# MachinaIO/mxx

Hardware: AMD Instinct MI355X
Metric: dcrt_ring_ops_per_s (higher is better)
Workload: dtype u32

## Files before the change

### mxx_amd/csrc/arith.hip

```cpp
#include "matmul_tile.h"

#include <algorithm>
#include <vector>

enum { OP_ADD = 0, OP_SUB = 1, OP_MUL = 2, OP_NEG = 3 };

template <typename W, int OP, bool BCAST, int VN>
__global__ void elementwise_kernel(W *__restrict__ out, const W *__restrict__ a, const W *__restrict__ b,
                                   const LimbConst *__restrict__ limbs, uint32_t L, uint32_t logN,
                                   size_t words_per_poly, size_t total_vecs) {
    size_t v = static_cast<size_t>(blockIdx.x) * blockDim.x + threadIdx.x;
    const size_t stride = static_cast<size_t>(gridDim.x) * blockDim.x;
    for (; v < total_vecs; v += stride) {
        const size_t w0 = v * VN;
        const uint32_t limb = static_cast<uint32_t>((w0 >> logN) % L);
        const LimbConst lc = limbs[limb];
        const W q = static_cast<W>(lc.q);
        const size_t bw0 = BCAST ? (w0 % words_per_poly) : w0;
        W av[VN], bv[VN], ov[VN];
        if (VN == 1) {
            av[0] = a[w0];
            bv[0] = b[bw0];
        } else {
            typedef typename std::conditional<sizeof(W) == 4, uint4, ulonglong2>::type V16;
// ... 439 lines not shown
            if (rc >= 0) return rc;
        }
        const bool want_dma = force ? (force == 'd' || force == 'w') : (rows32 && cols >= 16);
        if (want_dma) {
            const int rc = launch_matmul_dma_u32(out, lhs, rhs);
            if (rc >= 0) return rc;
        }
        const uint64_t lds_blocks = static_cast<uint64_t>(matrix_limbs(out)) * (N / 64) * ((cols + 15) / 16);
        const bool thin = rows <= 2 && cols >= 8 &&
                          lds_blocks <= 512 && (inner >= 128 || (rows >= 2 && inner >= 64));
        const bool want_lds = force ? (force == 'l' || force == 'd' || force == 'w') : ((rows >= 9 && cols >= 8 && !narrow) || thin);
        if (lds_ok && want_lds) return launch_matmul_lds_u32(out, lhs, rhs);
    }
    if (N >= 4) {
        switch (ctx->env.matmul_tile) {
#define MXX_TILE(R, C, S)                                                                   \
    case (R * 100 + C * 10 + S) * 2: return launch_matmul_cfg<uint32_t, R, C, S>(out, lhs, rhs); \
    case (R * 100 + C * 10 + S) * 2 + 1: return launch_matmul_cfg<uint32_t, R, C, S, true>(out, lhs, rhs);
            MXX_TILE(1, 8, 4) MXX_TILE(1, 4, 4) MXX_TILE(2, 8, 4) MXX_TILE(2, 4, 4) MXX_TILE(3, 4, 4) MXX_TILE(4, 4, 4)
            MXX_TILE(3, 8, 2) MXX_TILE(4, 8, 1) MXX_TILE(8, 8, 1) MXX_TILE(4, 8, 2)
#undef MXX_TILE
            default: break;
        }
        if (rows > 4 && rows <= 8) return launch_matmul_cfg<uint32_t, 8, 8, 1>(out, lhs, rhs);
        if (rows >= 4) {
            const uint64_t waves4 = static_cast<uint64_t>((N + 63) / 64) * ((cols + 7) / 8) * matrix_limbs(out);
            return waves4 <= 8192 ? launch_matmul_cfg<uint32_t, 4, 8, 1, true>(out, lhs, rhs) : launch_matmul_cfg<uint32_t, 4, 8, 1>(out, lhs, rhs);
        }
        if (rows == 3) {
            const uint64_t waves3 = static_cast<uint64_t>((N / 4 + 63) / 64) * ((cols + 3) / 4) * matrix_limbs(out);
            return waves3 <= 4096 ? launch_matmul_cfg<uint32_t, 3, 4, 4, true>(out, lhs, rhs) : launch_matmul_cfg<uint32_t, 3, 4, 4>(out, lhs, rhs);
        }
        const uint32_t tc = (rows >= 2 || cols >= 8) ? 8 : 4;
        const uint64_t tile_waves = static_cast<uint64_t>((N / 4 + 63) / 64) * ((rows + 1) / 2) * ((cols + tc - 1) / tc) * matrix_limbs(out);
        const bool ahead = tile_waves <= (rows >= 2 ? 1024u : 8192u);
        if (rows >= 2) return ahead ? launch_matmul_cfg<uint32_t, 2, 8, 4, true>(out, lhs, rhs) : launch_matmul_cfg<uint32_t, 2, 8, 4>(out, lhs, rhs);
        if (cols >= 8) {
            const int rc = launch_matmul_skinny24(out, lhs, rhs, ahead);
            if (rc >= 0) return rc;
        }
        if (cols >= 8) return ahead ? launch_matmul_cfg<uint32_t, 1, 8, 4, true>(out, lhs, rhs) : launch_matmul_cfg<uint32_t, 1, 8, 4>(out, lhs, rhs);
        return ahead ? launch_matmul_cfg<uint32_t, 1, 4, 4, true>(out, lhs, rhs) : launch_matmul_cfg<uint32_t, 1, 4, 4>(out, lhs, rhs);
    }
    return launch_matmul_cfg<uint32_t, 1, 4, 1>(out, lhs, rhs);
}

template <typename W, int OP, bool BCAST>
static int launch_elementwise_typed(GpuMatrix *out, const GpuMatrix *a, const GpuMatrix *b) {
    GpuContext *ctx = out->ctx;
    const size_t words = matrix_words(out);
    if (words == 0) return 0;
    const size_t wpp = matrix_limbs(out) * static_cast<size_t>(ctx->N);
    const uint32_t L = static_cast<uint32_t>(matrix_limbs(out));
    constexpr int VNATIVE = 16 / sizeof(W);
    MXX_TRACE_BYTES(static_cast<double>(words) * sizeof(W) * (1 + (OP == OP_NEG || BCAST || a == b ? 1 : 2)));
    if (ctx->N >= VNATIVE) {
        const size_t vecs = words / VNATIVE;
        unsigned blocks = static_cast<unsigned>(std::min<size_t>((vecs + 255) / 256, 16384));
        MXX_LAUNCH((elementwise_kernel<W, OP, BCAST, VNATIVE>), dim3(blocks), dim3(256), 0, ctx->stream,
                           static_cast<W *>(words_ptr(out)), static_cast<const W *>(words_ptr(a)),
                           static_cast<const W *>(words_ptr(b)), ctx->d_limbs, L, ctx->logN, wpp, vecs);
    } else {
        unsigned blocks = static_cast<unsigned>(std::min<size_t>((words + 255) / 256, 16384));
        MXX_LAUNCH((elementwise_kernel<W, OP, BCAST, 1>), dim3(blocks), dim3(256), 0, ctx->stream,
                           static_cast<W *>(words_ptr(out)), static_cast<const W *>(words_ptr(a)),
                           static_cast<const W *>(words_ptr(b)), ctx->d_limbs, L, ctx->logN, wpp, words);
    }
// ... 203 lines not shown
    if (out->ctx != lhs->ctx || out->ctx != rhs->ctx) return set_error(std::string(who) + ": context mismatch");
    if (out->level != lhs->level || out->level != rhs->level) return set_error(std::string(who) + ": level mismatch");
    if (mode != 0 && (base_bits == 0 || base_bits >= 63)) return set_error(std::string(who) + ": invalid base_bits");
    if (identity_size == 0) return set_error(std::string(who) + ": identity_size must be positive");
    if (storage_overlaps(out, lhs) || storage_overlaps(out, rhs)) return set_error(std::string(who) + ": output must not alias an input");
    GpuContext *ctx = out->ctx;
    const size_t L = matrix_limbs(out);
    const size_t dpt = mode == 0 ? 1 : (ctx->crt_bits + base_bits - 1) / base_bits;
    const size_t k = mode == 0 ? 1 : (mode == 1 ? dpt * L : dpt);
    const size_t w = rhs->rows * k;
    if (lhs->cols != w * identity_size || out->rows != lhs->rows || out->cols != rhs->cols * identity_size)
        return set_error(std::string(who) + ": shape mismatch");
    if (lhs->format != GPU_POLY_FORMAT_EVAL || (mode == 0 && rhs->format != GPU_POLY_FORMAT_EVAL))
        return set_error(std::string(who) + " requires Eval format");
    out->format = GPU_POLY_FORMAT_EVAL;
    if (matrix_polys(out) == 0) return 0;
    if (ctx_activate(ctx)) return 1;
    if (w == 0) {
        HIP_TRY(hipMemsetAsync(words_ptr(out), 0, out->bytes, ctx->stream));
        return 0;
    }
    const size_t poly_bytes = L * static_cast<size_t>(ctx->N) * ctx->word_bytes;
    size_t chunk = rhs->cols;
    if (mode != 0) {
        size_t free_b = 0, total_b = 0, budget = size_t(8) << 30;
        if (hipMemGetInfo(&free_b, &total_b) == hipSuccess) budget = std::max(budget, (free_b + ctx->cached_bytes) / 3);
        else (void)hipGetLastError();
        chunk = std::min(rhs->cols, std::max<size_t>(1, budget / (w * poly_bytes)));
    }
    const bool row_vector = lhs->rows == 1;
    const bool in_place = row_vector || (identity_size == 1 && chunk == rhs->cols);
    GpuMatrix *lhs_buf = nullptr, *prod = nullptr;
    int rc = 0;
    if (!row_vector && identity_size > 1) rc = gpu_matrix_create(ctx, out->level, lhs->rows, w, GPU_POLY_FORMAT_EVAL, &lhs_buf);
    if (!rc && !in_place) rc = gpu_matrix_create(ctx, out->level, lhs->rows, chunk, GPU_POLY_FORMAT_EVAL, &prod);
    for (size_t c0 = 0; !rc && c0 < rhs->cols; c0 += chunk) {
        const size_t cw = std::min(chunk, rhs->cols - c0);
        const bool whole = cw == rhs->cols;
        GpuMatrix *slice = nullptr, *dec = nullptr;
        if (!whole) {
            rc = gpu_matrix_create(ctx, out->level, rhs->rows, cw, rhs->format, &slice);
            if (!rc) rc = gpu_matrix_copy_block(slice, rhs, 0, 0, 0, c0, rhs->rows, cw);
        }
        const GpuMatrix *x = whole ? rhs : slice;
        if (!rc && mode != 0) {
            rc = gpu_matrix_create(ctx, out->level, w, cw, GPU_POLY_FORMAT_EVAL, &dec);
            if (!rc) rc = mode == 1 ? gpu_matrix_decompose_base(x, base_bits, dec) : gpu_matrix_decompose_base_small(x, base_bits, dec);
            x = dec;
        }
        for (size_t i = 0; !rc && i < identity_size; ++i) {
            GpuMatrix lhs_view = matrix_view(lhs, i * w, 1, w, poly_bytes);
            const GpuMatrix *a = lhs;
            if (row_vector) a = &lhs_view;
            else if (identity_size > 1) {
                rc = gpu_matrix_copy_block(lhs_buf, lhs, 0, 0, 0, i * w, lhs->rows, w);
                a = lhs_buf;
            }
            if (rc) break;
            if (row_vector) {
                GpuMatrix out_view = matrix_view(out, i * rhs->cols + c0, 1, cw, poly_bytes);
                rc = gpu_matrix_mul(&out_view, a, x);
            } else if (in_place) {
                rc = gpu_matrix_mul(out, a, x);
            } else {
                GpuMatrix prod_view = matrix_view(prod, 0, lhs->rows, cw, poly_bytes);
                rc = gpu_matrix_mul(&prod_view, a, x);
                if (!rc) rc = gpu_matrix_copy_block(out, &prod_view, 0, i * rhs->cols + c0, 0, 0, lhs->rows, cw);
            }
        }
        gpu_matrix_destroy(slice);
// ... 354 lines not shown
```

### mxx_amd/csrc/common.h

```cpp
#pragma once

#include <hip/hip_runtime.h>

#include <atomic>
#include <cstddef>
#include <cstdint>
#include <cstdio>
#include <exception>
#include <map>
#include <unordered_map>
#include <mutex>
#include <string>
#include <vector>

#include "../../include/gpupoly.h"

constexpr size_t GPUPOLY_MAX_LIMBS = 64;

struct LimbConst {
    uint64_t q;
    uint64_t mu;
    uint64_t mu64;
    uint64_t n_inv;
    uint64_t n_inv_sh;
// ... 2 lines not shown
    uint64_t inv_last_w_sh;
    uint32_t kbits;
    uint32_t lazy_terms;
};

struct EnvSwitches {
    int ntt_path = 0;
    int ntt14 = 0;
    bool decompose_fused = true;
    char matmul_path = 0;
    int matmul_tile = 0;
    bool gsamp_simple = false;
    bool gsamp_no_uni = false;
    bool p1_simple = false;
    int sampler_per_lane = 0;
    int sampler_fill_every = 0;
    bool ntt64_int = false;
    int ntt_phase = 0;
    bool serde_general = false;
    bool rng_compat = false;
    bool pack24 = true;
    int skinny24 = 0;
    int skinny24_shape = 0;
    size_t mul_decompose_many_budget = 0;
    size_t mul_decompose_pairs_budget = 0;
    size_t gadget_scalar_budget = 0;
    char mul_sum_path = 0;
    size_t crt_recompose_chunk_bytes = size_t(256) << 20;
    void load();
};

struct GpuContext {
    EnvSwitches env;
    int device = 0;
    std::vector<int> gpu_ids;
    uint32_t logN = 0;
    int N = 0;
    int level = 0;
    uint32_t dnum = 0;
    int limb_count = 0;
    bool wide = false;
    int word_bytes = 4;
    uint32_t crt_bits = 0;
    std::vector<uint64_t> moduli;
    hipStream_t stream = nullptr;
    LimbConst *d_limbs = nullptr;
// ... 30 lines not shown
};

struct LayoutTag {
    std::atomic<int> v{GPU_MATRIX_LAYOUT_WORDS};
    LayoutTag() = default;
    LayoutTag(const LayoutTag &o) : v(o.v.load(std::memory_order_acquire)) {}
    LayoutTag &operator=(const LayoutTag &o) {
        v.store(o.v.load(std::memory_order_acquire), std::memory_order_release);
        return *this;
    }
};

struct GpuMatrix {
    GpuContext *ctx = nullptr;
    int level = 0;
    size_t rows = 0, cols = 0;
    int format = GPU_POLY_FORMAT_EVAL;
    void *storage = nullptr;
    size_t bytes = 0;
    LayoutTag layout;
    bool borrowed = false;
    GpuMatrix *parent = nullptr;
    int views = 0;
};

struct GpuEventSet {
    std::vector<hipEvent_t> events;
    int device = 0;
    void *staging = nullptr;
    GpuContext *ctx = nullptr;
    void *dev_staging = nullptr;
};

struct GpuP1CovarianceCache {
    GpuContext *ctx = nullptr;
    int level = 0;
    size_t d = 0, m = 0, n = 0;
    double sigma = 0, s = 0, dgg_stddev = 0;
    double *sqrt_var = nullptr;
    double *update_coeff = nullptr;
    void *karney_div = nullptr;
};

struct P1KeyEntry {
    const double *sqrt_var;
    const double *update_coeff;
// ... 150 lines not shown
    void *release() {
        void *p = ptr;
        ptr = nullptr;
        return p;
    }
};
int matrix_check_same_shape(const GpuMatrix *a, const GpuMatrix *b, const char *who);
int coeff_domain_source(const GpuMatrix *mat, CtxBlock &scratch, const void **src);

int launch_ntt(GpuContext *ctx, void *data, size_t vectors, int limbs_per_poly, bool inverse);
int launch_ntt_lds_u32(GpuContext *ctx, uint32_t *data, size_t vectors, uint32_t L, bool inverse);
int launch_ntt_digits_u32(GpuContext *ctx, uint32_t *out, const uint32_t *coeff, size_t out_vectors, uint32_t L,
                          uint32_t src_cols, uint32_t towers, uint32_t dpt, uint32_t base_bits, size_t k, uint32_t td0 = 0);
int launch_ntt_lds_u64(GpuContext *ctx, uint64_t *data, size_t vectors, uint32_t L, bool inverse);
int launch_ntt_digits_u64(GpuContext *ctx, uint64_t *out, const uint64_t *coeff, size_t out_vectors, uint32_t L,
                          uint32_t src_cols, uint32_t towers, uint32_t dpt, uint32_t base_bits, size_t k, uint32_t td0 = 0);
int launch_intt_oop_u32(GpuContext *ctx, uint32_t *out, const uint32_t *in, size_t vectors, uint32_t L);
int launch_ntt_add_u32(GpuContext *ctx, uint32_t *out, const uint32_t *src, const uint32_t *add, size_t vectors, uint32_t L);
int launch_mul_intt_u32(GpuContext *ctx, uint32_t *out, const uint32_t *in, const uint32_t *w, size_t vectors, uint32_t L);
int launch_matmul(GpuMatrix *out, const GpuMatrix *lhs, const GpuMatrix *rhs);
int launch_ntt_fwd_pack24_u32(GpuContext *ctx, uint32_t *out, const uint32_t *in, size_t vectors, uint32_t L);
int launch_matmul_skinny24(GpuMatrix *out, const GpuMatrix *lhs, const GpuMatrix *rhs, bool small_grid);
int skinny24_parse_shape(const char *s);
int launch_matmul_dma_u32(GpuMatrix *out, const GpuMatrix *lhs, const GpuMatrix *rhs);
int launch_matmul_dma32_u32(GpuMatrix *out, const GpuMatrix *lhs, const GpuMatrix *rhs);
int launch_matmul_mfma_u32(GpuMatrix *out, const GpuMatrix *lhs, const GpuMatrix *rhs);
int launch_copy_block(GpuMatrix *out, const GpuMatrix *src, size_t dst_row, size_t dst_col, size_t src_row,
                      size_t src_col, size_t rows, size_t cols, bool add);
int sample_p1_keyed_segments(const GpuP1CovarianceCache *cache, const P1KeyEntry *d_keys, const GpuMatrix *tp2,
                             const GpuRngSeed *seeds, const size_t *seg_cols, size_t nseg, GpuMatrix *out);
int launch_scatter_i64(GpuMatrix *out, const int64_t *vals);
```

### mxx_amd/csrc/decompose.hip

```cpp
#include "common.h"
#include "modarith.h"

#include <algorithm>

static inline uint32_t host_bits(uint64_t v) { return v ? 64 - (uint32_t)__builtin_clzll(v) : 0; }

template <typename W>
__global__ void decompose_kernel(W *__restrict__ out, const W *__restrict__ src, const LimbConst *__restrict__ limbs,
                                 size_t src_polys, uint32_t src_cols, uint32_t L, uint32_t N, uint32_t towers,
                                 uint32_t dpt, uint32_t base_bits, size_t k) {
    const size_t idx = item_index();
    const size_t total = src_polys * towers * N;
    if (idx >= total) return;
    const uint32_t i = static_cast<uint32_t>(idx % N);
    const size_t pt = idx / N;
    const uint32_t t = static_cast<uint32_t>(pt % towers);
    const size_t p = pt / towers;
    const size_t r = p / src_cols, c = p - r * src_cols;
    const uint64_t residue = static_cast<uint64_t>(src[(p * L + t) * N + i]);
    const uint32_t src_bits = limbs[t].kbits;
    for (uint32_t d = 0; d < dpt; ++d) {
        const uint32_t shift = d * base_bits;
        uint64_t mask = 0;
        if (shift < src_bits) {
// ... 144 lines not shown

static int decompose_window(GpuContext *ctx, void *out, const void *coeff, size_t cols, size_t L, size_t k, uint32_t towers,
                            uint32_t dpt, uint32_t base_bits, size_t row_start, size_t R, bool eval) {
    const size_t row_bytes = cols * L * static_cast<size_t>(ctx->N) * static_cast<size_t>(ctx->word_bytes);
    char *o = static_cast<char *>(out);
    const char *c = static_cast<const char *>(coeff);
    const size_t first = row_start % k;
    size_t done = 0;
    if (first || R < k) {
        const size_t ky = std::min(R, k - first);
        if (int rc = decompose_segment(ctx, o, c, 1, cols, L, k, towers, dpt, base_bits, ky, static_cast<uint32_t>(first), eval)) return rc;
        done = ky;
        c += row_bytes;
    }
    if (const size_t whole = (R - done) / k) {
        if (int rc = decompose_segment(ctx, o + done * row_bytes, c, whole, cols, L, k, towers, dpt, base_bits, k, 0, eval)) return rc;
        done += whole * k;
        c += whole * row_bytes;
    }
    if (done < R) return decompose_segment(ctx, o + done * row_bytes, c, 1, cols, L, k, towers, dpt, base_bits, R - done, 0, eval);
    return 0;
}

static int decompose_core(const GpuMatrix *src, uint32_t base_bits, bool small, size_t row_start, GpuMatrix *out) {
    GpuContext *ctx = src->ctx;
    const int requested = out->format;
    const size_t L = matrix_limbs(src), R = out->rows, cols = src->cols;
    const uint32_t dpt = (ctx->crt_bits + base_bits - 1) / base_bits;
    const size_t k = small ? dpt : static_cast<size_t>(dpt) * L;
    if (R == 0 || cols == 0) {
        out->format = GPU_POLY_FORMAT_EVAL;
        return 0;
    }
    if (ctx_activate(ctx)) return 1;
    const size_t r0 = row_start / k, nsrc = (row_start + R - 1) / k - r0 + 1;
    const size_t row_bytes = cols * L * static_cast<size_t>(ctx->N) * static_cast<size_t>(ctx->word_bytes);
    const void *coeff = static_cast<const char *>(words_ptr(src)) + r0 * row_bytes;
    CtxBlock tmp_block(ctx);
    if (src->format == GPU_POLY_FORMAT_EVAL) {
        const size_t bytes = nsrc * row_bytes;
        if (tmp_block.alloc(bytes)) return 1;
        int rc = ctx->wide ? -1 : launch_intt_oop_u32(ctx, static_cast<uint32_t *>(tmp_block.ptr), static_cast<const uint32_t *>(coeff),
                                                      nsrc * cols * L, static_cast<uint32_t>(L));
        if (rc < 0) {
            MXX_TRACED_COPY("copy (device to device)", ctx->stream, 2.0 * bytes,
                            HIP_TRY(hipMemcpyAsync(tmp_block.ptr, coeff, bytes, hipMemcpyDeviceToDevice, ctx->stream)));
            rc = launch_ntt(ctx, tmp_block.ptr, nsrc * cols * L, static_cast<int>(L), true);
        }
        if (rc) return rc;
        coeff = tmp_block.ptr;
    }
    const uint32_t towers = small ? 1u : static_cast<uint32_t>(L);
    const bool eval = requested == GPU_POLY_FORMAT_EVAL;
    const int rc = decompose_window(ctx, words_ptr(out), coeff, cols, L, k, towers, dpt, base_bits, row_start - r0 * k, R, eval);
    if (rc == 0) out->format = eval ? GPU_POLY_FORMAT_EVAL : GPU_POLY_FORMAT_COEFF;
    return rc;
}

static int decompose_impl(const GpuMatrix *src, uint32_t base_bits, GpuMatrix *out, bool small) {
    if (!src || !out) return set_error("gpu_matrix_decompose_base: null matrix");
    if (base_bits == 0) return set_error("base_bits must be non-zero in gpu_matrix_decompose_base");
    if (src->ctx != out->ctx || src->level != out->level)
        return set_error("context mismatch in gpu_matrix_decompose_base");
    if (storage_overlaps(src, out)) return set_error("gpu_matrix_decompose_base: output must not alias the source");
    const size_t L = matrix_limbs(src);
    const uint32_t dpt = (src->ctx->crt_bits + base_bits - 1) / base_bits;
    const size_t k = small ? dpt : static_cast<size_t>(dpt) * L;
    if (out->rows != src->rows * k || out->cols != src->cols)
        return set_error("output size mismatch in gpu_matrix_decompose_base");
    return decompose_core(src, base_bits, small, 0, out);
}

extern "C" int gpu_matrix_fill_gadget(GpuMatrix *out, uint32_t base_bits) {
    ABI_GUARD_BEGIN
    return fill_gadget_impl(out, base_bits, false);
    ABI_GUARD_END
}

extern "C" int gpu_matrix_fill_small_gadget(GpuMatrix *out, uint32_t base_bits) {
    ABI_GUARD_BEGIN
    return fill_gadget_impl(out, base_bits, true);
    ABI_GUARD_END
}

extern "C" int gpu_matrix_decompose_base(const GpuMatrix *src, uint32_t base_bits, GpuMatrix *out) {
    ABI_GUARD_BEGIN
    return decompose_impl(src, base_bits, out, false);
    ABI_GUARD_END
}

extern "C" int gpu_matrix_decompose_base_small(const GpuMatrix *src, uint32_t base_bits, GpuMatrix *out) {
    ABI_GUARD_BEGIN
    return decompose_impl(src, base_bits, out, true);
// ... 198 lines not shown
```

### mxx_amd/csrc/layout.hip

```cpp
#include "common.h"

#include <stdexcept>

namespace {

__global__ void __launch_bounds__(256) unpack24_kernel(uint4 *__restrict__ words, const uint32_t *__restrict__ packed, size_t groups) {
    const size_t g = item_index();
    if (g >= groups) return;
    const uint32_t *p = packed + 3 * g;
    const uint32_t w0 = __builtin_nontemporal_load(p), w1 = __builtin_nontemporal_load(p + 1), w2 = __builtin_nontemporal_load(p + 2);
    words[g] = make_uint4(w0 & 0xffffffu, __builtin_amdgcn_alignbit(w1, w0, 24) & 0xffffffu,
                          __builtin_amdgcn_alignbit(w2, w1, 16) & 0xffffffu, w2 >> 8);
}

typedef uint32_t u32x4 __attribute__((ext_vector_type(4)));
__global__ void __launch_bounds__(256) pack24_kernel(uint32_t *__restrict__ packed, const u32x4 *__restrict__ words, size_t groups) {
    const size_t g = item_index();
    if (g >= groups) return;
    const u32x4 w = __builtin_nontemporal_load(words + g);
    uint32_t *p = packed + 3 * g;
    p[0] = w.x | (w.y << 24);
    p[1] = (w.y >> 8) | (w.z << 16);
    p[2] = (w.z >> 16) | (w.w << 8);
}
// ... 49 lines not shown
    GpuContext *ctx = m->ctx;
    const uint32_t L = static_cast<uint32_t>(matrix_limbs(m));
    const size_t vectors = matrix_polys(m) * L;
    std::unique_lock<std::mutex> lk(ctx->layout_mutex);
    if (m->views) {
        lk.unlock();
        return ntt ? launch_ntt(ctx, m->storage, vectors, static_cast<int>(L), false) : 0;
    }
    CtxBlock packed(ctx);
    if (packed.alloc(packed24_bytes(m))) return 1;
    int rc = ntt ? launch_ntt_fwd_pack24_u32(ctx, static_cast<uint32_t *>(packed.ptr), static_cast<const uint32_t *>(m->storage), vectors, L) : -1;
    if (rc < 0) {
        if (ntt && (rc = launch_ntt(ctx, m->storage, vectors, static_cast<int>(L), false))) return rc;
        const size_t groups = m->bytes / 16;
        MXX_TRACE_BYTES(static_cast<double>(packed24_bytes(m)) + m->bytes);
        MXX_LAUNCH(pack24_kernel, item_grid(groups, 256), dim3(256), 0, ctx->stream, static_cast<uint32_t *>(packed.ptr),
                   static_cast<const u32x4 *>(m->storage), groups);
        HIP_TRY(hipGetLastError());
    } else if (rc) {
        return rc;
    }
    ctx_free(ctx, m->storage);
    m->storage = packed.release();
    m->layout.v.store(GPU_MATRIX_LAYOUT_PACKED24, std::memory_order_release);
    return 0;
}
```

### mxx_amd/csrc/ntt14.h

```cpp
#pragma once

#include "ntt_lds.h"

namespace ntt14 {
constexpr int LOGN = 14;
constexpr uint32_t N = 1u << LOGN;
constexpr uint32_t T = 512;
constexpr int R0 = 32;
constexpr uint32_t BLK = 512;
constexpr uint32_t BLK_PAD = BLK + 64;
constexpr uint32_t GROUP_WORDS = 8 * BLK_PAD;

__device__ __forceinline__ uint32_t pad64(uint32_t pos) { return pos + ((pos >> 5) << 2); }

__device__ __forceinline__ void wave_sync() {
    __builtin_amdgcn_fence(__ATOMIC_ACQ_REL, "wavefront");
    __builtin_amdgcn_wave_barrier();
}

#ifdef GPUPOLY_PHASE_TIMING
#define NTT14_PHASE(bit) ((phase & (bit)) != 0)
#else
#define NTT14_PHASE(bit) false
#endif
// ... 187 lines not shown

template <typename W, bool TIGHT = false>
__global__ void __launch_bounds__(512, 8 / (sizeof(W) / 4))
    fwd_add_kernel(W *__restrict__ out, const W *__restrict__ src, const W *__restrict__ add,
                   const TwPair<W> *__restrict__ tw_all, const LimbConst *__restrict__ limbs, uint32_t L) {
    const uint32_t limb = blockIdx.x;
    const size_t vec = (static_cast<size_t>(blockIdx.z) * gridDim.y + blockIdx.y) * L + limb;
    const LimbConst lc = limbs[limb];
    fwd_body<W, TIGHT, true, LoadVector<W, true>, true, true>(out + vec * N, LoadVector<W, true>{src + vec * N}, tw_all, lc, limb, add + vec * N);
}

template <typename W, bool REDUCE>
struct LoadDigit {
    const W *src;
    uint32_t shift;
    W mask, q;
    __device__ __forceinline__ W operator()(uint32_t e) const {
        const W digit = (src[e] >> shift) & mask;
        if constexpr (REDUCE) return digit >= q ? digit % q : digit;
        else return digit;
    }
};

template <typename W, bool REDUCE, bool TIGHT = false, bool NTS = false>
__global__ void __launch_bounds__(512, 8 / (sizeof(W) / 4))
    fwd_digits_kernel(W *__restrict__ out, const W *__restrict__ coeff, const TwPair<W> *__restrict__ tw_all,
                      const LimbConst *__restrict__ limbs, uint32_t L, uint32_t src_cols, uint32_t towers, uint32_t dpt,
                      uint32_t base_bits, uint32_t k, uint32_t td0) {
    const uint32_t rest = blockIdx.x >> 3, col_hi = rest / L, limb = rest - col_hi * L;
    const uint32_t col = col_hi * 8u + (blockIdx.x & 7u);
    if (col >= src_cols) return;
    const uint32_t td = blockIdx.y + td0;
    const size_t r = blockIdx.z;
    const uint32_t t = td / dpt, d = td - t * dpt;
    const size_t vec = ((r * k + blockIdx.y) * src_cols + col) * L + limb;
    const LimbConst lc = limbs[limb];
    const uint32_t src_bits = limbs[t].kbits, shift = d * base_bits;
    LoadDigit<W, REDUCE> load;
    load.src = coeff + ((r * src_cols + col) * L + t) * N;
    load.shift = shift < 8 * sizeof(W) ? shift : 0;
    load.mask = 0;
    if (shift < src_bits && shift < 8 * sizeof(W)) {
        const uint32_t rem = src_bits - shift;
        const uint32_t db = base_bits < rem ? base_bits : rem;
        load.mask = db >= 8 * sizeof(W) ? static_cast<W>(~static_cast<W>(0)) : static_cast<W>((static_cast<W>(1) << db) - 1);
    }
    load.q = static_cast<W>(lc.q);
    (void)towers;
    fwd_body<W, TIGHT, NTS, LoadDigit<W, REDUCE>, false, NTS>(out + vec * N, load, tw_all, lc, limb);
}

template <typename W, bool SGN, bool MULW = false, int CAP = 31, int WPS = ((SGN && !MULW) ? 8 : 6), bool NT = false>
__global__ void __launch_bounds__(512, WPS / (sizeof(W) / 4))
    inv_kernel(W *__restrict__ data, const TwPair<W> *__restrict__ tw_all, const LimbConst *__restrict__ limbs,
               uint32_t L, const W *in = nullptr, const W *__restrict__ mulw = nullptr) {
    extern __shared__ __attribute__((aligned(16))) unsigned char smem[];
    W *xs = reinterpret_cast<W *>(smem);
    typedef typename std::conditional<sizeof(W) == 4, uint4, ulonglong2>::type V16;
    constexpr int VN = 16 / sizeof(W);
    const uint32_t tid = threadIdx.x, lane = tid & 63u;
    const uint32_t wave = __builtin_amdgcn_readfirstlane(tid >> 6);
    const uint32_t limb = blockIdx.x;
    const size_t vec = (static_cast<size_t>(blockIdx.z) * gridDim.y + blockIdx.y) * L + limb;
    const LimbConst lc = limbs[limb];
    const W q = static_cast<W>(lc.q);
    const W muw = static_cast<W>(sizeof(W) == 4 ? lc.mu32 : lc.mu64);
    const TwPair<W> *tw = tw_all + static_cast<size_t>(limb) * N;
    W *g = data + vec * N;
    const W *gin = (!MULW && in) ? in + vec * N : g;

    V16 dnext[8 / VN], wnext[8 / VN];
    const W *src0 = (MULW ? in + vec * N : g) + wave * BLK + 8 * lane;
// ... 95 lines not shown
```

### mxx_amd/csrc/ntt_lds_u32.hip

```cpp
#include "ntt_rings.h"

using W = uint32_t;

int launch_ntt_lds_u32(GpuContext *ctx, uint32_t *data, size_t vectors, uint32_t L, bool inverse) {
    return launch_ntt_lds<W>(ctx, data, vectors, L, inverse);
}

template __global__ void ntt14::inv_kernel<W, true, false, 31, 8, true>(W *, const TwPair<W> *, const LimbConst *, uint32_t, const W *,
                                                                        const W *);

template <typename R, bool TIGHT>
static int launch_lazy_mulw(GpuContext *ctx, W *out, const W *in, const W *w, size_t vectors, uint32_t L) {
    const size_t lds = R::template lds<W>();
    if (lds > kLdsLimitBytes) return -1;
    if (int rc = lds_opt_in<ntt_inv_lazy_kernel<W, R::LOGN, R::LOGR, R::WPE, 0, TIGHT, false, true>>(ctx, lds)) return rc;
    MXX_LAUNCH((ntt_inv_lazy_kernel<W, R::LOGN, R::LOGR, R::WPE, 0, TIGHT, false, true>), dim3(static_cast<unsigned>(vectors)), R::block(),
               lds, ctx->stream, out, tw_inv<W>(ctx), ctx->d_limbs_r, L, in, w);
    HIP_TRY(hipGetLastError());
    return 0;
}

template <typename R, bool TIGHT>
static int launch_split_mulw(GpuContext *ctx, W *out, const W *in, const W *w, size_t vectors, uint32_t L) {
    const size_t lds = R::template lds<W>();
// ... 59 lines not shown
    MXX_TRACE_BYTES(3.0 * vectors * ntt14::N * sizeof(W));
    return bool_dispatch(!ctx->lazy_ok, [&](auto TIGHT) {
        MXX_LAUNCH((ntt14::fwd_add_kernel<W, TIGHT()>), grid, dim3(ntt14::T), ntt14::lds_bytes(sizeof(W)), ctx->stream, out, src, add,
                   tw_fwd<W>(ctx), ctx->d_limbs, L);
        HIP_TRY(hipGetLastError());
        return 0;
    });
}

int launch_ntt_digits_u32(GpuContext *ctx, uint32_t *out, const uint32_t *coeff, size_t out_vectors, uint32_t L,
                          uint32_t src_cols, uint32_t towers, uint32_t dpt, uint32_t base_bits, size_t k, uint32_t td0) {
    DigitLaunch<W> d{out, coeff, L, src_cols, towers, dpt, base_bits, 0, td0};
    if (!ntt14_switches(ctx, true, true) || !d.plan(ctx, out_vectors, k)) return -1;
    MXX_TRACE_BYTES((static_cast<double>(d.src_rows) * src_cols * L + static_cast<double>(out_vectors)) * ctx->N * sizeof(W));
    if (ctx->logN != 14) return launch_ntt_digits<W>(ctx, d);
    const dim3 grid(8u * L * ((src_cols + 7u) / 8u), d.k, static_cast<unsigned>(d.src_rows));
    return bool_dispatch(d.reduce, !ctx->lazy_ok, d.nts, [&](auto RED, auto TIGHT, auto NTS) {
        MXX_LAUNCH((ntt14::fwd_digits_kernel<W, RED(), TIGHT(), NTS()>), grid, dim3(ntt14::T), ntt14::lds_bytes(sizeof(W)), ctx->stream, out,
                   coeff, tw_fwd<W>(ctx), ctx->d_limbs, L, src_cols, towers, dpt, base_bits, d.k, td0);
        HIP_TRY(hipGetLastError());
        return 0;
    });
}
```

### mxx_amd/csrc/runtime.hip

```cpp
#include "common.h"

#include <algorithm>
#include <cstdlib>
#include <iterator>
#include <map>
#include <cstring>
#include <dlfcn.h>

typedef unsigned __int128 u128h;

static thread_local std::string g_last_error;

int set_error(const char *msg) {
    g_last_error = msg ? msg : "unknown error";
    return 1;
}
int set_error(const std::string &msg) {
    g_last_error = msg;
    return 1;
}
int set_error(hipError_t err, const char *what) {
    g_last_error = std::string(what ? what : "hip call") + ": " + hipGetErrorString(err);
    (void)hipGetLastError();
    return 1;
// ... 223 lines not shown
    }
    if (const char *e = std::getenv("MXX_HIP_NTT14")) ntt14 = e[0] == 'w' ? 1 : (e[0] == 'u' ? 2 : 0);
    if (const char *e = std::getenv("MXX_HIP_DECOMPOSE_FUSED")) decompose_fused = e[0] != '0';
    if (const char *e = std::getenv("MXX_HIP_MATMUL_PATH")) matmul_path = e[0];
    if (const char *e = std::getenv("MXX_HIP_MATMUL_TILE")) {
        if (e[0] && e[1] && e[2]) matmul_tile = ((e[0] - '0') * 100 + (e[1] - '0') * 10 + (e[2] - '0')) * 2 + (e[3] == 'p');
    }
    if (const char *e = std::getenv("MXX_HIP_GSAMP")) {
        gsamp_simple = e[0] == 's';
        gsamp_no_uni = e[0] == 'n';
    }
    if (const char *e = std::getenv("MXX_HIP_P1")) p1_simple = e[0] == 's';
    if (const char *e = std::getenv("MXX_HIP_NTT64")) ntt64_int = e[0] == 'i';
    if (const char *e = std::getenv("MXX_HIP_RNG_COMPAT")) rng_compat = e[0] == 'r';
    if (const char *e = std::getenv("MXX_HIP_SERDE")) serde_general = e[0] == 'g';
    if (const char *e = std::getenv("MXX_HIP_PACK24")) pack24 = !(std::strcmp(e, "0") == 0 || std::strcmp(e, "off") == 0);
    if (const char *e = std::getenv("MXX_HIP_SKINNY24")) {
        if (std::strcmp(e, "0") == 0) skinny24 = 1;
        else if (std::strncmp(e, "force", 5) == 0 && (e[5] == 0 || e[5] == ':')) {
            skinny24 = 2;
            if (e[5] == ':') skinny24_shape = skinny24_parse_shape(e + 6) ? skinny24_parse_shape(e + 6) : -1;
        }
    }
    if (const char *e = std::getenv("MXX_HIP_MUL_DECOMPOSE_MANY_BUDGET")) mul_decompose_many_budget = static_cast<size_t>(std::strtoull(e, nullptr, 10));
    if (const char *e = std::getenv("MXX_HIP_MUL_DECOMPOSE_PAIRS_BUDGET")) mul_decompose_pairs_budget = static_cast<size_t>(std::strtoull(e, nullptr, 10));
    if (const char *e = std::getenv("MXX_HIP_GADGET_SCALAR_BUDGET")) gadget_scalar_budget = static_cast<size_t>(std::strtoull(e, nullptr, 10));
    if (const char *e = std::getenv("MXX_HIP_CRT_RECOMPOSE_CHUNK_BYTES")) {
        const size_t v = static_cast<size_t>(std::strtoull(e, nullptr, 10));
        if (v >= 1) crt_recompose_chunk_bytes = v;
    }
    if (const char *e = std::getenv("MXX_HIP_MUL_SUM_PATH")) mul_sum_path = (e[0] == 't' || e[0] == 's') ? e[0] : 0;
    if (const char *e = std::getenv("MXX_HIP_SAMPLER_PER_LANE")) {
        const int v = std::atoi(e);
        if (v >= 1 && v <= 4096) sampler_per_lane = v;
    }
    if (const char *e = std::getenv("MXX_HIP_NTT_PHASE")) {
        const int v = std::atoi(e);
        if (v >= 0 && v <= 127) ntt_phase = v;
    }
    if (const char *e = std::getenv("MXX_HIP_SAMPLER_FILL_EVERY")) {
        const int v = std::atoi(e);
        if (v >= 1 && v <= 8) sampler_fill_every = v;
    }
}

static std::mutex g_registry_mutex;
// ... 523 lines not shown
```

Baseline: 7.788 million.

## Emit decomposed digits in packed 24-bit layout and add few-row packed matmul kernel

In mul_decompose, the forward NTT of gadget digits now writes its output straight into a packed 3-byte-per-residue layout when the following matmul will read packed B, instead of producing full u32 digits that are later repacked. A new fewrow24 matmul kernel handles 4-8 row LHS against packed24 RHS, using either unaligned loads or ds_bpermute unpacking, with optional XCD-aware block remapping. The goal is to cut digit-matrix memory traffic and allocation by a quarter, allow larger chunks, and skip a separate pack pass. It adds considerable code and extra lane-shuffle work in the inner loop.

```diff
diff --git a/mxx_amd/csrc/arith.hip b/mxx_amd/csrc/arith.hip
--- a/mxx_amd/csrc/arith.hip
+++ b/mxx_amd/csrc/arith.hip
@@ -485,6 +485,10 @@
 #undef MXX_TILE
             default: break;
         }
+        if (rows >= 4 && rows <= 8) {
+            const int rc = launch_matmul_fewrow24(out, lhs, rhs);
+            if (rc >= 0) return rc;
+        }
         if (rows > 4 && rows <= 8) return launch_matmul_cfg<uint32_t, 8, 8, 1>(out, lhs, rhs);
         if (rows >= 4) {
             const uint64_t waves4 = static_cast<uint64_t>((N + 63) / 64) * ((cols + 7) / 8) * matrix_limbs(out);
@@ -506,6 +510,14 @@
         return ahead ? launch_matmul_cfg<uint32_t, 1, 4, 4, true>(out, lhs, rhs) : launch_matmul_cfg<uint32_t, 1, 4, 4>(out, lhs, rhs);
     }
     return launch_matmul_cfg<uint32_t, 1, 4, 1>(out, lhs, rhs);
+}
+
+bool matmul_reads_packed_b(const GpuContext *ctx, size_t rows, size_t inner, size_t cols, size_t L) {
+    const size_t N = static_cast<size_t>(ctx->N);
+    if (ctx->wide || ctx->env.matmul_path || ctx->env.matmul_tile || N < 64 || N % 64 || rows == 0 || rows > 8) return false;
+    const uint64_t lds_blocks = static_cast<uint64_t>(L) * (N / 64) * ((cols + 15) / 16);
+    const bool thin = rows <= 2 && cols >= 8 && lds_blocks <= 512 && (inner >= 128 || (rows >= 2 && inner >= 64));
+    return !thin;
 }
 
 template <typename W, int OP, bool BCAST>
@@ -755,11 +767,15 @@
     }
     const size_t poly_bytes = L * static_cast<size_t>(ctx->N) * ctx->word_bytes;
     size_t chunk = rhs->cols;
+    bool packed_d = false;
     if (mode != 0) {
         size_t free_b = 0, total_b = 0, budget = size_t(8) << 30;
         if (hipMemGetInfo(&free_b, &total_b) == hipSuccess) budget = std::max(budget, (free_b + ctx->cached_bytes) / 3);
         else (void)hipGetLastError();
-        chunk = std::min(rhs->cols, std::max<size_t>(1, budget / (w * poly_bytes)));
+        packed_d = !ctx->wide && ctx->pack24_ok && ctx->env.pack24 && (ctx->env.digits24 & 3) != 1 && ctx->logN == 14 &&
+                   matmul_reads_packed_b(ctx, lhs->rows, w, rhs->cols, L);
+        const size_t d_poly_bytes = packed_d ? poly_bytes / 4 * 3 : poly_bytes;
+        chunk = std::min(rhs->cols, std::max<size_t>(1, budget / (w * d_poly_bytes)));
     }
     const bool row_vector = lhs->rows == 1;
     const bool in_place = row_vector || (identity_size == 1 && chunk == rhs->cols);
@@ -777,8 +793,13 @@
         }
         const GpuMatrix *x = whole ? rhs : slice;
         if (!rc && mode != 0) {
-            rc = gpu_matrix_create(ctx, out->level, w, cw, GPU_POLY_FORMAT_EVAL, &dec);
-            if (!rc) rc = mode == 1 ? gpu_matrix_decompose_base(x, base_bits, dec) : gpu_matrix_decompose_base_small(x, base_bits, dec);
+            int prc = -1;
+            if (packed_d && matmul_reads_packed_b(ctx, lhs->rows, w, cw, L)) prc = decompose_base_packed24(x, base_bits, mode == 2, &dec);
+            if (prc >= 0) rc = prc;
+            else {
+                rc = gpu_matrix_create(ctx, out->level, w, cw, GPU_POLY_FORMAT_EVAL, &dec);
+                if (!rc) rc = mode == 1 ? gpu_matrix_decompose_base(x, base_bits, dec) : gpu_matrix_decompose_base_small(x, base_bits, dec);
+            }
             x = dec;
         }
         for (size_t i = 0; !rc && i < identity_size; ++i) {
diff --git a/mxx_amd/csrc/common.h b/mxx_amd/csrc/common.h
--- a/mxx_amd/csrc/common.h
+++ b/mxx_amd/csrc/common.h
@@ -48,6 +48,7 @@
     bool pack24 = true;
     int skinny24 = 0;
     int skinny24_shape = 0;
+    int digits24 = 0;
     size_t mul_decompose_many_budget = 0;
     size_t mul_decompose_pairs_budget = 0;
     size_t gadget_scalar_budget = 0;
@@ -124,6 +125,7 @@
     bool borrowed = false;
     GpuMatrix *parent = nullptr;
     int views = 0;
+    bool padded24 = false;
 };
 
 struct GpuEventSet {
@@ -320,6 +322,11 @@
 int launch_ntt_fwd_pack24_u32(GpuContext *ctx, uint32_t *out, const uint32_t *in, size_t vectors, uint32_t L);
 int launch_matmul_skinny24(GpuMatrix *out, const GpuMatrix *lhs, const GpuMatrix *rhs, bool small_grid);
 int skinny24_parse_shape(const char *s);
+int launch_matmul_fewrow24(GpuMatrix *out, const GpuMatrix *lhs, const GpuMatrix *rhs);
+bool matmul_reads_packed_b(const GpuContext *ctx, size_t rows, size_t inner, size_t cols, size_t L);
+int launch_ntt_digits_pack24_u32(GpuContext *ctx, uint32_t *out, const uint32_t *coeff, size_t out_vectors, uint32_t L,
+                                 uint32_t src_cols, uint32_t towers, uint32_t dpt, uint32_t base_bits, size_t k, bool probe);
+int decompose_base_packed24(const GpuMatrix *src, uint32_t base_bits, bool small, GpuMatrix **out);
 int launch_matmul_dma_u32(GpuMatrix *out, const GpuMatrix *lhs, const GpuMatrix *rhs);
 int launch_matmul_dma32_u32(GpuMatrix *out, const GpuMatrix *lhs, const GpuMatrix *rhs);
 int launch_matmul_mfma_u32(GpuMatrix *out, const GpuMatrix *lhs, const GpuMatrix *rhs);
diff --git a/mxx_amd/csrc/decompose.hip b/mxx_amd/csrc/decompose.hip
--- a/mxx_amd/csrc/decompose.hip
+++ b/mxx_amd/csrc/decompose.hip
@@ -190,6 +190,26 @@
     return 0;
 }
 
+static int coeff_rows(const GpuMatrix *src, size_t r0, size_t nsrc, CtxBlock &scratch, const void **coeff) {
+    GpuContext *ctx = src->ctx;
+    const size_t L = matrix_limbs(src), cols = src->cols;
+    const size_t row_bytes = cols * L * static_cast<size_t>(ctx->N) * static_cast<size_t>(ctx->word_bytes);
+    *coeff = static_cast<const char *>(words_ptr(src)) + r0 * row_bytes;
+    if (src->format != GPU_POLY_FORMAT_EVAL) return 0;
+    const size_t bytes = nsrc * row_bytes;
+    if (scratch.alloc(bytes)) return 1;
+    int rc = ctx->wide ? -1 : launch_intt_oop_u32(ctx, static_cast<uint32_t *>(scratch.ptr), static_cast<const uint32_t *>(*coeff),
+                                                  nsrc * cols * L, static_cast<uint32_t>(L));
+    if (rc < 0) {
+        MXX_TRACED_COPY("copy (device to device)", ctx->stream, 2.0 * bytes,
+                        HIP_TRY(hipMemcpyAsync(scratch.ptr, *coeff, bytes, hipMemcpyDeviceToDevice, ctx->stream)));
+        rc = launch_ntt(ctx, scratch.ptr, nsrc * cols * L, static_cast<int>(L), true);
+    }
+    if (rc) return rc;
+    *coeff = scratch.ptr;
+    return 0;
+}
+
 static int decompose_core(const GpuMatrix *src, uint32_t base_bits, bool small, size_t row_start, GpuMatrix *out) {
     GpuContext *ctx = src->ctx;
     const int requested = out->format;
@@ -202,22 +222,9 @@
     }
     if (ctx_activate(ctx)) return 1;
     const size_t r0 = row_start / k, nsrc = (row_start + R - 1) / k - r0 + 1;
-    const size_t row_bytes = cols * L * static_cast<size_t>(ctx->N) * static_cast<size_t>(ctx->word_bytes);
-    const void *coeff = static_cast<const char *>(words_ptr(src)) + r0 * row_bytes;
+    const void *coeff = nullptr;
     CtxBlock tmp_block(ctx);
-    if (src->format == GPU_POLY_FORMAT_EVAL) {
-        const size_t bytes = nsrc * row_bytes;
-        if (tmp_block.alloc(bytes)) return 1;
-        int rc = ctx->wide ? -1 : launch_intt_oop_u32(ctx, static_cast<uint32_t *>(tmp_block.ptr), static_cast<const uint32_t *>(coeff),
-                                                      nsrc * cols * L, static_cast<uint32_t>(L));
-        if (rc < 0) {
-            MXX_TRACED_COPY("copy (device to device)", ctx->stream, 2.0 * bytes,
-                            HIP_TRY(hipMemcpyAsync(tmp_block.ptr, coeff, bytes, hipMemcpyDeviceToDevice, ctx->stream)));
-            rc = launch_ntt(ctx, tmp_block.ptr, nsrc * cols * L, static_cast<int>(L), true);
-        }
-        if (rc) return rc;
-        coeff = tmp_block.ptr;
-    }
+    if (int rc = coeff_rows(src, r0, nsrc, tmp_block, &coeff)) return rc;
     const uint32_t towers = small ? 1u : static_cast<uint32_t>(L);
     const bool eval = requested == GPU_POLY_FORMAT_EVAL;
     const int rc = decompose_window(ctx, words_ptr(out), coeff, cols, L, k, towers, dpt, base_bits, row_start - r0 * k, R, eval);
@@ -237,6 +244,46 @@
     if (out->rows != src->rows * k || out->cols != src->cols)
         return set_error("output size mismatch in gpu_matrix_decompose_base");
     return decompose_core(src, base_bits, small, 0, out);
+}
+
+int decompose_base_packed24(const GpuMatrix *src, uint32_t base_bits, bool small, GpuMatrix **out) {
+    *out = nullptr;
+    GpuContext *ctx = src->ctx;
+    if (ctx->wide || !ctx->env.pack24 || (ctx->env.digits24 & 3) == 1) return -1;
+    const size_t L = matrix_limbs(src), cols = src->cols;
+    const uint32_t dpt = (ctx->crt_bits + base_bits - 1) / base_bits;
+    const size_t k = small ? dpt : static_cast<size_t>(dpt) * L;
+    const uint32_t towers = small ? 1u : static_cast<uint32_t>(L);
+    const size_t out_vectors = src->rows * k * cols * L;
+    if (out_vectors == 0 || cols >> 32 ||
+        launch_ntt_digits_pack24_u32(ctx, nullptr, nullptr, out_vectors, static_cast<uint32_t>(L), static_cast<uint32_t>(cols), towers, dpt,
+                                     base_bits, k, true) < 0)
+        return -1;
+    if (ctx_activate(ctx)) return 1;
+    const void *coeff = nullptr;
+    CtxBlock tmp_block(ctx);
+    if (int rc = coeff_rows(src, 0, src->rows, tmp_block, &coeff)) return rc;
+    GpuMatrix *m = new GpuMatrix();
+    m->ctx = ctx;
+    m->level = src->level;
+    m->rows = src->rows * k;
+    m->cols = cols;
+    m->format = GPU_POLY_FORMAT_EVAL;
+    m->bytes = matrix_words(m) * static_cast<size_t>(ctx->word_bytes);
+    if (ctx_alloc(ctx, packed24_bytes(m) + 16, &m->storage)) {
+        delete m;
+        return 1;
+    }
+    m->padded24 = true;
+    m->layout.v.store(GPU_MATRIX_LAYOUT_PACKED24, std::memory_order_release);
+    const int rc = launch_ntt_digits_pack24_u32(ctx, static_cast<uint32_t *>(m->storage), static_cast<const uint32_t *>(coeff), out_vectors,
+                                                static_cast<uint32_t>(L), static_cast<uint32_t>(cols), towers, dpt, base_bits, k, false);
+    if (rc) {
+        gpu_matrix_destroy(m);
+        return rc < 0 ? set_error("gpupoly_matrix_mul_decompose: the packed digit transform refused a launch it had accepted") : rc;
+    }
+    *out = m;
+    return 0;
 }
 
 extern "C" int gpu_matrix_fill_gadget(GpuMatrix *out, uint32_t base_bits) {
diff --git a/mxx_amd/csrc/layout.hip b/mxx_amd/csrc/layout.hip
--- a/mxx_amd/csrc/layout.hip
+++ b/mxx_amd/csrc/layout.hip
@@ -95,6 +95,7 @@
     }
     ctx_free(ctx, m->storage);
     m->storage = packed.release();
+    m->padded24 = false;
     m->layout.v.store(GPU_MATRIX_LAYOUT_PACKED24, std::memory_order_release);
     return 0;
 }
diff --git a/mxx_amd/csrc/matmul_fewrow24.hip b/mxx_amd/csrc/matmul_fewrow24.hip
--- /dev/null
+++ b/mxx_amd/csrc/matmul_fewrow24.hip
@@ -0,0 +1,160 @@
+#include "common.h"
+#include "matmul_tile.h"
+#include "modarith.h"
+
+#include <string>
+
+namespace fewrow24 {
+
+typedef uint32_t u32_unaligned __attribute__((aligned(1)));
+
+template <int TR, bool NTB, int LD>
+__global__ void __launch_bounds__(256)
+    kernel(uint32_t *__restrict__ C, const uint32_t *__restrict__ A, const unsigned char *__restrict__ B, const LimbConst *__restrict__ limbs,
+           uint32_t rows, uint32_t inner, uint32_t cols, uint32_t L, uint32_t N, uint32_t col_tiles, uint32_t share) {
+    constexpr int TC = 8;
+    uint32_t limb, bx, by;
+    if (share) {
+        const uint32_t xcd = blockIdx.x & 7u, j = blockIdx.x >> 3, xblocks = N / 256u;
+        by = j % col_tiles;
+        const uint32_t group = (j / col_tiles) * 8u + xcd;
+        limb = group / xblocks;
+        bx = group - limb * xblocks;
+    } else {
+        limb = blockIdx.z;
+        bx = blockIdx.x;
+        by = blockIdx.y;
+    }
+    const uint32_t rt = by / col_tiles, ct = by - rt * col_tiles;
+    const uint32_t r0 = rt * TR, c0 = ct * TC;
+    const uint32_t i = bx * blockDim.x + threadIdx.x;
+    const LimbConst lc = limbs[limb];
+    const uint32_t q = static_cast<uint32_t>(lc.q);
+    const uint32_t lane = threadIdx.x & 63u;
+
+    const size_t strideA = static_cast<size_t>(L) * N;
+    size_t a_off[TR], b_off[TC];
+#pragma unroll
+    for (int r = 0; r < TR; ++r) {
+        const uint32_t rr = min(r0 + r, rows - 1);
+        a_off[r] = (static_cast<size_t>(rr) * inner * L + limb) * N + i;
+    }
+    const uint32_t lane_off = LD == 0 ? i * 3u : (i - lane) * 3u + min(lane, 47u) * 4u;
+#pragma unroll
+    for (int c = 0; c < TC; ++c) {
+        const uint32_t cc = min(c0 + c, cols - 1);
+        b_off[c] = (static_cast<size_t>(cc) * L + limb) * N * 3 + lane_off;
+    }
+    const size_t strideBk = static_cast<size_t>(cols) * L * N * 3;
+    const uint32_t d = (lane * 3u) >> 2, sh = ((lane * 3u) & 3u) * 8u;
+    const int sel_lo = static_cast<int>(d * 4u), sel_hi = static_cast<int>(min(d + 1u, 47u) * 4u);
+
+    uint64_t acc[TR][TC];
+#pragma unroll
+    for (int r = 0; r < TR; ++r)
+#pragma unroll
+        for (int c = 0; c < TC; ++c) acc[r][c] = 0;
+    const uint32_t lazy = lc.lazy_terms;
+    uint32_t pending = 0;
+    for (uint32_t k = 0; k < inner; ++k) {
+        uint32_t av[TR], bv[TC];
+#pragma unroll
+        for (int r = 0; r < TR; ++r) av[r] = A[a_off[r] + k * strideA];
+#pragma unroll
+        for (int c = 0; c < TC; ++c) {
+            const unsigned char *p = B + b_off[c] + k * strideBk;
+            if constexpr (LD == 0) {
+                const u32_unaligned *src = reinterpret_cast<const u32_unaligned *>(p);
+                if constexpr (NTB) bv[c] = __builtin_nontemporal_load(src);
+                else bv[c] = *src;
+            } else {
+                const uint32_t *src = reinterpret_cast<const uint32_t *>(p);
+                if constexpr (NTB) bv[c] = __builtin_nontemporal_load(src);
+                else bv[c] = *src;
+            }
+        }
+#pragma unroll
+        for (int c = 0; c < TC; ++c) {
+            if constexpr (LD == 0) {
+                bv[c] &= 0xffffffu;
+            } else {
+                const uint32_t lo = static_cast<uint32_t>(__builtin_amdgcn_ds_bpermute(sel_lo, static_cast<int>(bv[c])));
+                const uint32_t hi = static_cast<uint32_t>(__builtin_amdgcn_ds_bpermute(sel_hi, static_cast<int>(bv[c])));
+                bv[c] = __builtin_amdgcn_alignbit(hi, lo, sh) & 0xffffffu;
+            }
+        }
+#pragma unroll
+        for (int r = 0; r < TR; ++r)
+#pragma unroll
+            for (int c = 0; c < TC; ++c) acc[r][c] += static_cast<uint64_t>(av[r]) * static_cast<uint64_t>(bv[c]);
+        if (++pending == lazy) {
+            pending = 0;
+#pragma unroll
+            for (int r = 0; r < TR; ++r)
+#pragma unroll
+                for (int c = 0; c < TC; ++c) acc[r][c] = reduce_u64_sum(acc[r][c], q, lc.mu64);
+        }
+    }
+#pragma unroll
+    for (int r = 0; r < TR; ++r) {
+        if (r0 + r >= rows) continue;
+#pragma unroll
+        for (int c = 0; c < TC; ++c) {
+            if (c0 + c >= cols) continue;
+            C[((static_cast<size_t>(r0 + r) * cols + (c0 + c)) * L + limb) * N + i] = reduce_u64_sum(acc[r][c], q, lc.mu64);
+        }
+    }
+}
+
+constexpr int kDefaultLoader = 1;
+
+}
+
+int launch_matmul_fewrow24(GpuMatrix *out, const GpuMatrix *lhs, const GpuMatrix *rhs) {
+    using namespace fewrow24;
+    GpuContext *ctx = out->ctx;
+    const EnvSwitches &env = ctx->env;
+    const int form = env.digits24 & 3;
+    if (form == 1 || ctx->wide || lhs->ctx != ctx || rhs->ctx != ctx) return -1;
+    const uint32_t rows = static_cast<uint32_t>(lhs->rows), inner = static_cast<uint32_t>(lhs->cols), cols = static_cast<uint32_t>(rhs->cols);
+    const uint32_t L = static_cast<uint32_t>(matrix_limbs(out)), N = static_cast<uint32_t>(ctx->N);
+    if (lhs->rows < 4 || lhs->rows > 8 || N % 256 != 0) return -1;
+    if (rhs->layout.v.load(std::memory_order_acquire) != GPU_MATRIX_LAYOUT_PACKED24) return -1;
+    const bool tall = rows > 4;
+    if (!tile_grid_fits(rows, cols, tall ? 8 : 4, 8)) return set_error("gpu_matrix_mul: matrix too large");
+    const TileGrid g = tall ? tile_grid<8, 8, 1>(ctx, rows, cols, L, rhs->bytes) : tile_grid<4, 8, 1>(ctx, rows, cols, L, rhs->bytes);
+    const int ld = rhs->padded24 ? (form == 2 ? 0 : (form == 3 ? 1 : kDefaultLoader)) : 1;
+    uint32_t *c = static_cast<uint32_t *>(words_ptr(out));
+    if (lhs->layout.v.load(std::memory_order_acquire) == GPU_MATRIX_LAYOUT_PACKED24) (void)words_ptr(lhs);
+    std::lock_guard<std::mutex> lk(ctx->layout_mutex);
+    bool pa = false, pb = false;
+    const uint32_t *a = static_cast<const uint32_t *>(packed24_ptr(lhs, &pa));
+    const unsigned char *b = static_cast<const unsigned char *>(packed24_ptr(rhs, &pb));
+    if (pa || !pb) return -1;
+    auto label = [](int key) {
+        const int tr = key & 4 ? 8 : 4, ld_ = key & 1;
+        const bool nt = key & 2;
+        return "fewrow24::kernel<TR=" + std::to_string(tr) + (nt ? ",nt" : "") + (ld_ ? ",bpermute" : ",unaligned") +
+               ",packed24 B> (the tile of matmul_kernel<u32," + std::to_string(tr) + ",8,1>, one slot per lane, 3-byte residues, " +
+               (ld_ ? "48 aligned dwords per wave through ds_bpermute" : "one unaligned dword per lane") +
+               (nt ? ", B streamed once with non-temporal loads)" : ")");
+    };
+    static const std::string name[8] = {label(0), label(1), label(2), label(3), label(4), label(5), label(6), label(7)};
+    const int key = (tall ? 4 : 0) | (g.streamed ? 2 : 0) | ld;
+    MXX_TRACE_BYTES(static_cast<double>(lhs->bytes) + packed24_bytes(rhs) + out->bytes);
+    const uint64_t blocks = static_cast<uint64_t>(g.grid.x) * g.grid.y * g.grid.z;
+    const uint32_t share = (env.digits24 & 4) == 0 && g.col_tiles > 1 && (static_cast<uint64_t>(L) * (N / 256u)) % 8 == 0 && blocks <= 0x7fffffffull;
+    const dim3 grid = share ? dim3(static_cast<unsigned>(blocks)) : g.grid;
+#define MXX_FR(KEY_)                                                                                                                        \
+    case KEY_:                                                                                                                          \
+        MXX_LAUNCH((kernel<(KEY_ & 4 ? 8 : 4), (KEY_ & 2) != 0, (KEY_ & 1)>), grid, dim3(g.threads), 0, ctx->stream, c, a, b, ctx->d_limbs, \
+                   rows, inner, cols, L, N, g.col_tiles, share);                                                                       \
+        break;
+    switch (key) {
+        MXX_FR(0) MXX_FR(1) MXX_FR(2) MXX_FR(3) MXX_FR(4) MXX_FR(5) MXX_FR(6) MXX_FR(7)
+    }
+#undef MXX_FR
+    ctx->last_kernel = name[key].c_str();
+    HIP_TRY(hipGetLastError());
+    return 0;
+}
diff --git a/mxx_amd/csrc/ntt14.h b/mxx_amd/csrc/ntt14.h
--- a/mxx_amd/csrc/ntt14.h
+++ b/mxx_amd/csrc/ntt14.h
@@ -233,7 +233,7 @@
     }
 };
 
-template <typename W, bool REDUCE, bool TIGHT = false, bool NTS = false>
+template <typename W, bool REDUCE, bool TIGHT = false, bool NTS = false, bool PK = false>
 __global__ void __launch_bounds__(512, 8 / (sizeof(W) / 4))
     fwd_digits_kernel(W *__restrict__ out, const W *__restrict__ coeff, const TwPair<W> *__restrict__ tw_all,
                       const LimbConst *__restrict__ limbs, uint32_t L, uint32_t src_cols, uint32_t towers, uint32_t dpt,
@@ -258,7 +258,7 @@
     }
     load.q = static_cast<W>(lc.q);
     (void)towers;
-    fwd_body<W, TIGHT, NTS, LoadDigit<W, REDUCE>, false, NTS>(out + vec * N, load, tw_all, lc, limb);
+    fwd_body<W, TIGHT, NTS, LoadDigit<W, REDUCE>, false, NTS, false, PK>(out + vec * (PK ? N / 4 * 3 : N), load, tw_all, lc, limb);
 }
 
 template <typename W, bool SGN, bool MULW = false, int CAP = 31, int WPS = ((SGN && !MULW) ? 8 : 6), bool NT = false>
diff --git a/mxx_amd/csrc/ntt_lds_u32.hip b/mxx_amd/csrc/ntt_lds_u32.hip
--- a/mxx_amd/csrc/ntt_lds_u32.hip
+++ b/mxx_amd/csrc/ntt_lds_u32.hip
@@ -105,3 +105,18 @@
         return 0;
     });
 }
+
+int launch_ntt_digits_pack24_u32(GpuContext *ctx, uint32_t *out, const uint32_t *coeff, size_t out_vectors, uint32_t L,
+                                 uint32_t src_cols, uint32_t towers, uint32_t dpt, uint32_t base_bits, size_t k, bool probe) {
+    DigitLaunch<W> d{nullptr, coeff, L, src_cols, towers, dpt, base_bits, 0, 0};
+    if (ctx->logN != 14 || !ctx->pack24_ok || !ctx->lazy_ok || !ntt14_switches(ctx, false, true) || !d.plan(ctx, out_vectors, k)) return -1;
+    if (probe) return 0;
+    MXX_TRACE_BYTES((static_cast<double>(d.src_rows) * src_cols * L + 0.75 * static_cast<double>(out_vectors)) * ctx->N * sizeof(W));
+    const dim3 grid(8u * L * ((src_cols + 7u) / 8u), d.k, static_cast<unsigned>(d.src_rows));
+    return bool_dispatch(d.reduce, d.nts, [&](auto RED, auto NTS) {
+        MXX_LAUNCH((ntt14::fwd_digits_kernel<W, RED(), false, NTS(), true>), grid, dim3(ntt14::T), ntt14::lds_bytes(sizeof(W)), ctx->stream, out,
+                   coeff, tw_fwd<W>(ctx), ctx->d_limbs, L, src_cols, towers, dpt, base_bits, d.k, 0u);
+        HIP_TRY(hipGetLastError());
+        return 0;
+    });
+}
diff --git a/mxx_amd/csrc/runtime.hip b/mxx_amd/csrc/runtime.hip
--- a/mxx_amd/csrc/runtime.hip
+++ b/mxx_amd/csrc/runtime.hip
@@ -269,6 +269,8 @@
             if (e[5] == ':') skinny24_shape = skinny24_parse_shape(e + 6) ? skinny24_parse_shape(e + 6) : -1;
         }
     }
+    if (const char *e = std::getenv("MXX_HIP_DIGITS24"))
+        digits24 = (std::strcmp(e, "0") == 0 ? 1 : (e[0] == 'u' ? 2 : (e[0] == 'b' ? 3 : 0))) | (std::strstr(e, "+grid") ? 4 : 0);
     if (const char *e = std::getenv("MXX_HIP_MUL_DECOMPOSE_MANY_BUDGET")) mul_decompose_many_budget = static_cast<size_t>(std::strtoull(e, nullptr, 10));
     if (const char *e = std::getenv("MXX_HIP_MUL_DECOMPOSE_PAIRS_BUDGET")) mul_decompose_pairs_budget = static_cast<size_t>(std::strtoull(e, nullptr, 10));
     if (const char *e = std::getenv("MXX_HIP_GADGET_SCALAR_BUDGET")) gadget_scalar_budget = static_cast<size_t>(std::strtoull(e, nullptr, 10));
```

New measurement: 7.783 million. No clear change (-0.1%).
